# cnettel/cnF2freq

Measured on AMD Instinct MI355X. Metric: individual*marker fwd-bwd steps/sec (all 8 shift modes, forward+backward, dosage rows), higher is better.
Workload: dtype f64

## Files before the change

cnf2freq_amd/capi.py:

```python
import ctypes as C
import os

import numpy as np

_HERE = os.path.dirname(os.path.abspath(__file__))
LIB_PATH = os.environ.get("CNF2HIP_LIB") or os.path.join(_HERE, "libcnf2hip.so")

OUT_DEVICE, NO_DOSAGE, RAW_DOSAGE, NO_TIES, FULL_SPILL, MERGE_MODES, ACC_DEVICE, ACC_KEEP, XPOSE, LOG_PATHS = 1, 2, 4, 8, 16, 32, 64, 128, 256, 512
ACC_TABLE = 1024
ACC_LANES = 2048
TIES_GENERAL = 4096
UPDATE_PLAIN = 8192
UPDATE_BOTH_FLOWS = 1 << 16
UPDATE_ONE_SCOUT = 1 << 17
UPDATE_LITERAL_FINISH = 1 << 19
DETERMINISTIC = 16384
TURN_VALU = 32768
FLUSH_TINY = 1 << 20
ALL_STATES = 1 << 21
QTL_ADDITIVE = 1 << 22
QTL_ORIGIN_DEVICE = 1 << 23
QTL_REG_DEVICE = 1 << 28
QTL_IMPRINT = 1 << 25
QTL_STATE_DEVICE = 1 << 29
NO_UNIFORM_PACK = 1 << 26
NO_UNIFORM_PACK8 = 1 << 27
NO_LINE_RECORDS = 1 << 24
STATIC_JOBS = 1 << 18
MINFACTOR = float(np.float32(-1e15))
IGNORED = -1e30

SYMBOLS = [
    "cnf2_device_count", "cnf2_ctx_create", "cnf2_ctx_destroy", "cnf2_last_error", "cnf2_version",
    "cnf2_upload_map", "cnf2_upload_rows", "cnf2_update_rows", "cnf2_update_rows_device",
    "cnf2_upload_pedigree",
    "cnf2_window_info", "cnf2_sweep", "cnf2_sync", "cnf2_fwbw_store", "cnf2_locked_query",
    "cnf2_turn_scan", "cnf2_turn_scan_rows", "cnf2_state_posterior", "cnf2_haplos", "cnf2_infprobs", "cnf2_infprobs_rows", "cnf2_descendants", "cnf2_accumulate", "cnf2_sweep_accumulate", "cnf2_sweep_turn_scan", "cnf2_fixparents_scan", "cnf2_variances", "cnf2_variances_exact",
    "cnf2_snapshot_priors", "cnf2_update_pass", "cnf2_download_rows", "cnf2_download_accumulators", "cnf2_upload_accumulators", "cnf2_accumulator_ptrs", "cnf2_update_stats", "cnf2_update_stats_guided", "cnf2_addvariance", "cnf2_emission", "cnf2_emission_paths",
    "cnf2_selftest_lane_xor", "cnf2_last_kernel_ms", "cnf2_last_paths", "cnf2_workspace_bytes", "cnf2_reserve_accumulate", "cnf2_clock_probe", "cnf2_sweep_clock", "cnf2_stream",
    "cnf2_set_grid_reserve", "cnf2_set_batch_jobs", "cnf2_set_line_records", "cnf2_last_line_records", "cnf2_last_uniform_pack", "cnf2_last_uniform_pack8", "cnf2_window_table", "cnf2_update_pass_records", "cnf2_exchange_buffer", "cnf2_exchange_download", "cnf2_exchange_upload", "cnf2_exchange_read", "cnf2_exchange_write",
    "cnf2_packed_accumulator_doubles", "cnf2_packed_row_bytes", "cnf2_pack_accumulators", "cnf2_unpack_accumulators",
    "cnf2_pack_rows", "cnf2_unpack_rows",
    "cnf2_crossover_rows", "cnf2_sweep_crossovers", "cnf2_sweep_viterbi", "cnf2_sweep_sample",
    "cnf2_sweep_place", "cnf2_sweep_loo", "cnf2_loo_rows", "cnf2_sweep_origins", "cnf2_origin_rows",
    "cnf2_qtl_scan", "cnf2_sweep_qtl", "cnf2_set_qtl_columns", "cnf2_qtl_scan2", "cnf2_set_qtl2_columns", "cnf2_qtl_scanx", "cnf2_set_qtlx_columns",
    "cnf2_qtl_scan_em", "cnf2_set_qtlem_columns", "cnf2_qtl_scan_binary", "cnf2_set_qtlbin_columns",
    "cnf2_qtl_scan_surv", "cnf2_set_qtlsurv_columns", "cnf2_set_qtlsurv_blocks",
    "cnf2_qtl_scan_var", "cnf2_set_qtlvar_columns",
    "cnf2_qtl_scan_cof", "cnf2_set_qtlcof_columns", "cnf2_qtl_kept_rows",
    "cnf2_kinship_sums", "cnf2_qtl_scan_cols", "cnf2_qtl_scan_boot", "cnf2_qtl_scan_mv", "cnf2_set_qtlmv_groups",
    "cnf2_qtl_scan_imp", "cnf2_set_qtlimp_columns",
]


class Cnf2Error(RuntimeError):
    pass


_lib = None


def hip_runtimes():
    paths = set()
# ... 95 lines not shown
        L.cnf2_snapshot_priors.argtypes = [vp, vp]
        L.cnf2_update_pass.argtypes = [vp, i32, vp, vp, vp, vp, vp, C.c_double, C.c_double, vp, C.c_uint32]
        L.cnf2_download_rows.argtypes = [vp, i32, i32, vp, vp, vp]
        L.cnf2_download_accumulators.argtypes = [vp, vp, vp, vp]
        L.cnf2_upload_accumulators.argtypes = [vp, vp, vp, vp]
        L.cnf2_accumulator_ptrs.argtypes = [vp, vp, vp, vp]
        L.cnf2_update_stats.argtypes = [vp, vp]
        L.cnf2_update_stats_guided.argtypes = [vp, vp]
        L.cnf2_emission.argtypes = [vp, i32, i32, vp]
        L.cnf2_emission_paths.argtypes = [vp, i32, i32, vp]
        L.cnf2_selftest_lane_xor.argtypes = [vp, vp]
        L.cnf2_last_kernel_ms.argtypes = [vp, vp, i32]
        L.cnf2_last_paths.argtypes = [vp, vp, i32]
        L.cnf2_workspace_bytes.argtypes = [vp]
        L.cnf2_workspace_bytes.restype = C.c_size_t
        L.cnf2_clock_probe.argtypes = [vp, vp]
        L.cnf2_sweep_clock.argtypes = [vp, vp]
        L.cnf2_set_grid_reserve.argtypes = [vp, i32]
        L.cnf2_set_batch_jobs.argtypes = [vp, i32]
        L.cnf2_set_line_records.argtypes = [vp, i32]
        L.cnf2_last_line_records.argtypes = [vp, vp]
        L.cnf2_last_uniform_pack.argtypes = [vp, vp]
        L.cnf2_last_uniform_pack8.argtypes = [vp, vp]
        L.cnf2_window_table.argtypes = [vp, vp]
        L.cnf2_update_pass_records.argtypes = [vp, i32, vp, i32, vp, vp, C.c_double, C.c_double, vp, C.c_uint32]
        L.cnf2_exchange_buffer.argtypes = [vp, C.c_size_t, vp]
        L.cnf2_exchange_download.argtypes = [vp, vp, C.c_size_t]
        L.cnf2_exchange_upload.argtypes = [vp, vp, C.c_size_t]
        L.cnf2_exchange_read.argtypes = [vp, C.c_size_t, vp, C.c_size_t]
        L.cnf2_exchange_write.argtypes = [vp, C.c_size_t, vp, C.c_size_t]
        L.cnf2_packed_accumulator_doubles.argtypes = [vp]
        L.cnf2_packed_accumulator_doubles.restype = C.c_size_t
        L.cnf2_packed_row_bytes.argtypes = [vp]
        L.cnf2_packed_row_bytes.restype = C.c_size_t
        for f in (L.cnf2_pack_accumulators, L.cnf2_unpack_accumulators, L.cnf2_pack_rows, L.cnf2_unpack_rows):
            f.argtypes = [vp, vp, i32, vp]
        L.cnf2_stream.argtypes = [vp]
        L.cnf2_stream.restype = vp
        _lib = L
    return _lib


def _p(a):
    return a.ctypes.data_as(C.c_void_p)


# ... 131 lines not shown
        self._chk(self.L.cnf2_last_kernel_ms(self.h, _p(ms), 4), "cnf2_last_kernel_ms")
        return float(ms[0])

    def set_grid_reserve(self, blocks):
        self._chk(self.L.cnf2_set_grid_reserve(self.h, blocks), "cnf2_set_grid_reserve")

    def set_line_records(self, lines):
        self._chk(self.L.cnf2_set_line_records(self.h, lines), "cnf2_set_line_records")

    def last_line_records(self):
        out = np.zeros(4, np.int32)
        self._chk(self.L.cnf2_last_line_records(self.h, _p(out)), "cnf2_last_line_records")
        return dict(lines=int(out[0]), on_records=int(out[1]), fallback=int(out[2]), bytes=int(out[3]))

    def last_uniform_pack(self):
        out = np.zeros(2, np.int32)
        self._chk(self.L.cnf2_last_uniform_pack(self.h, _p(out)), "cnf2_last_uniform_pack")
        return dict(jobs=int(out[0]), groups=int(out[1]))

    def last_uniform_pack8(self):
        out = np.zeros(2, np.int32)
        self._chk(self.L.cnf2_last_uniform_pack8(self.h, _p(out)), "cnf2_last_uniform_pack8")
        return dict(eights=int(out[0]), jobs=int(out[1]))

    def set_batch_jobs(self, jobs):
        self._chk(self.L.cnf2_set_batch_jobs(self.h, jobs), "cnf2_set_batch_jobs")

    def workspace_bytes(self):
        return int(self.L.cnf2_workspace_bytes(self.h))

    def window_info(self, ind):
        out = np.zeros(17, np.int32)
        self._chk(self.L.cnf2_window_info(self.h, ind, _p(out)), "cnf2_window_info")
        return dict(shiftignore=int(out[0]), flag2ignore=int(out[1]), founder=int(out[2]),
                    slots=out[3:10].copy(), tie=out[10:17].copy())

    def fwbw_store(self, ind, chrom=0):
        mc = int(self.chromstarts[chrom + 1] - self.chromstarts[chrom])
        fw = np.zeros((8, mc, 3, 64))
        ff = np.zeros((8, mc, 3))
        self._chk(self.L.cnf2_fwbw_store(self.h, ind, chrom, _p(fw), _p(ff)), "cnf2_fwbw_store")
        return fw, ff

    def locked_query(self, ind, chrom, marker):
        v = np.zeros((8, 64, 128))
        self._chk(self.L.cnf2_locked_query(self.h, ind, chrom, marker, _p(v)), "cnf2_locked_query")
# ... 875 lines not shown
```

cnf2freq_amd/csrc/cnf2_capi.hip:

```cpp
#include "../../include/cnf2hip.h"

#include <hip/hip_runtime.h>
#include <math.h>
#include <cmath>
#include <stdarg.h>
#include <chrono>
#include <stdio.h>
#include <string.h>

#include <string>
#include <algorithm>
#include <vector>

#include "cnf2_device.h"
#include "cnf2_emission.h"
#include "cnf2_emtab.h"
#include "cnf2_plan.h"
#include "cnf2_qtl.h"
#include "cnf2_qtlplan.h"
#include "cnf2_qtl2.h"
#include "cnf2_qtlx.h"
#include "cnf2_qtlcof.h"
#include "cnf2_qtlem.h"
#include "cnf2_qtlbin.h"
// ... 76 lines not shown
    std::vector<Window> windows;
    DevBuf<Window>      d_windows;
    bool                windows_dirty = true;
    DevBuf<uint8_t>     d_rowflags;
    int                 fast_blocks_per_cu = 1;
    int                 uni_blocks_per_cu = 1;
    int                 reserve_blocks = 0;
    int                 batch_jobs = 0;

    int                  line_cap = -1;
    int32_t              last_lines[4] = {0, 0, 0, 0};
    int32_t              last_pack[2] = {0, 0};
    int32_t              last_pack8[2] = {0, 0};
    unsigned             windows_gen = 0;
    bool                 lines_valid = false;
    unsigned             lines_gen = 0;
    int                  lines_begin = 0, lines_n = 0, lines_cap = 0;
    int                  lines_fit = 1 << 30;
    std::vector<LineKey> h_lines;
    std::vector<int32_t> h_line_keys, h_line_hash;
    DevBuf<LineKey>      d_lines;
    DevBuf<int32_t>      d_line_keys;
    DevBuf<LineRec>      d_line_rec;

    DevBuf<Job>       d_jobs;
    DevBuf<PackedJob> d_pjobs;
    DevBuf<double>    d_spill;
    DevBuf<double>    d_factors, d_loglik, d_dosage;
    DevBuf<int32_t>   d_lexp;
    DevBuf<unsigned long long> d_clock;
    DevBuf<PackedJob> d_upjobs;
    DevBuf<int>       d_jobnext;
    DevBuf<double>    d_scratch;

    DevBuf<double>  d_xo_f;
    int             xo_blocks_per_cu = 1;
    DevBuf<double>  d_xo;
    DevBuf<double>  d_xo_sum;
    DevBuf<int32_t> d_xo_cnt;

    DevBuf<double>  d_vit_lm;
    DevBuf<uint8_t> d_vit_st;
    DevBuf<int32_t> d_vit_sh;

    DevBuf<uint8_t> d_smp_st;
    DevBuf<int32_t> d_smp_sh;
// ... 288 lines not shown

int cnf2_sync(cnf2_ctx* ctx)
{
    if (!ctx) return CNF2_ERR_ARG;
    HIP_TRY(ctx, hipStreamSynchronize(ctx->stream));
    return CNF2_OK;
}

int cnf2_upload_map(cnf2_ctx* ctx, const double* pos, int n_markers, const int32_t* chromstarts, int n_chrom,
                    const double* genrec)
{
    if (!ctx || !pos || !chromstarts || n_markers <= 0 || n_chrom <= 0) return fail(ctx, CNF2_ERR_ARG, "bad map arguments");
    if (chromstarts[0] != 0 || chromstarts[n_chrom] != n_markers)
        return fail(ctx, CNF2_ERR_ARG, "chromstarts must run from 0 to n_markers");
    for (int c = 0; c < n_chrom; c++)
        if (chromstarts[c + 1] <= chromstarts[c]) return fail(ctx, CNF2_ERR_ARG, "empty chromosome %d", c);
    HIP_TRY(ctx, hipSetDevice(ctx->device));
    if (ctx->n_markers != n_markers && (ctx->d_allele8 || ctx->d_sure || ctx->d_hw))
        return fail(ctx, CNF2_ERR_STATE, "marker count changed after rows were uploaded");
    ctx->qtl_rows_n = 0;
    ctx->n_markers = n_markers;
    ctx->n_chrom   = n_chrom;
    ctx->chromstarts.assign(chromstarts, chromstarts + n_chrom + 1);
    if (genrec) memcpy(ctx->genrec, genrec, sizeof(ctx->genrec));
    std::vector<double2> rho(n_markers);
    for (int m = 0; m < n_markers; m++) {
        double2 r = make_double2(0.0, 0.0);
        if (m + 1 < n_markers) {
            double dist = pos[m + 1] - pos[m];
            if (dist > 0) {
                r.x = 0.5 * (1.0 - exp(ctx->genrec[0] * dist));
                r.y = 0.5 * (1.0 - exp(ctx->genrec[1] * dist));
            }
        }
        rho[m] = r;
    }
    RC_TRY(ctx->d_rho.alloc(ctx, n_markers));
    HIP_TRY(ctx, hipMemcpy(ctx->d_rho, rho.data(), sizeof(double2) * n_markers, hipMemcpyHostToDevice));
    std::vector<double2> tq(n_markers);
    std::vector<double>  logk(n_chrom, 0.0);
    for (int c = 0; c < n_chrom; c++)
        for (int m = chromstarts[c]; m < chromstarts[c + 1]; m++) {
            tq[m] = make_double2(rho[m].x / (1.0 - rho[m].x), rho[m].y / (1.0 - rho[m].y));
            if (m + 1 < chromstarts[c + 1]) logk[c] += 4.0 * log1p(-rho[m].x) + 2.0 * log1p(-rho[m].y);
        }
    RC_TRY(ctx->d_tq.release(ctx));
// ... 335 lines not shown
        ctx->lines_n     = n;
        ctx->lines_cap   = cap;
        ctx->lines_valid = true;
    }
    *n_lines = (int)ctx->h_lines.size();
    return CNF2_OK;
}

static int sweep_impl(cnf2_ctx* ctx, int ind_begin, int ind_end, double* factors_out, double* loglik_out, double* dosage_out,
                      uint32_t flags, const SweepMode& mode)
{
    RC_TRY(ready(ctx));
    const int n_all = (int)ctx->windows.size();
    if (ind_begin < 0 || ind_end > n_all || ind_begin > ind_end) return fail(ctx, CNF2_ERR_ARG, "individual range out of bounds");
    const bool plain = mode.variant == SW_PLAIN;
    if (!plain) flags &= ~(uint32_t)(CNF2_MERGE_MODES | CNF2_XPOSE | CNF2_FLUSH_TINY | CNF2_NO_TIES | CNF2_RAW_DOSAGE);
    const bool want_dosage = !(flags & CNF2_NO_DOSAGE) && plain;
    if (!factors_out || !loglik_out || (want_dosage && !dosage_out)) return fail(ctx, CNF2_ERR_ARG, "output pointer is NULL");
    const int n = ind_end - ind_begin;
    if (n == 0) return CNF2_OK;
    HIP_TRY(ctx, hipSetDevice(ctx->device));

    if ((size_t)n * ctx->n_chrom > 0x7fffffff) return fail(ctx, CNF2_ERR_ARG, "too many jobs in one call");
    JobPlan      jp = job_plan(ctx, ind_begin, n, flags);
    const size_t n_fast = jp.n_fast, n_general = jp.jobs.size() - n_fast, n_packed = jp.pjobs.size();
    RC_TRY(ctx->d_jobs.ensure(ctx, jp.jobs.size() + 1));
    if (n_packed > 0) {
        RC_TRY(ctx->d_pjobs.ensure(ctx, n_packed));
        HIP_TRY(ctx, hipMemcpyAsync(ctx->d_pjobs, jp.pjobs.data(), sizeof(PackedJob) * n_packed, hipMemcpyHostToDevice, ctx->stream));
    }
    std::vector<PackedJob> ugroups;
    const std::vector<Job> jobs_planned = jp.jobs;
    auto group_and_upload = [&](const int32_t* keys) -> int {
        jp.jobs = jobs_planned;
        ugroups.clear();
        size_t n_single = n_fast;
        if (keys && !(flags & CNF2_NO_UNIFORM_PACK))
            ugroups = group_uniform_jobs(jp.jobs, n_fast, ctx->windows.data() + ind_begin, keys, &n_single);
        if (!jp.jobs.empty())
            HIP_TRY(ctx, hipMemcpyAsync(ctx->d_jobs, jp.jobs.data(), sizeof(Job) * jp.jobs.size(), hipMemcpyHostToDevice, ctx->stream));
        HIP_TRY(ctx, hipStreamSynchronize(ctx->stream));
        return CNF2_OK;
    };

    const int    mlen = longest_chrom(ctx);
    const size_t stride = spill_stride(mlen);
    int          grid_fast = 0, grid_gen = 0;
    size_t       free_b = 0, total_b = 0;
    HIP_TRY(ctx, hipMemGetInfo(&free_b, &total_b));
    size_t n_uniform = 0, n_on_records = 0;
    int    n_lines = 0;
    const bool uni_ok = !(flags & (CNF2_ALL_STATES | CNF2_FULL_SPILL | CNF2_XPOSE)) && (plain || mode.variant == SW_VITERBI);
    const int  want_lines = ctx->line_cap >= 0 ? std::min(ctx->line_cap, ctx->lines_fit) : ctx->lines_fit;
    auto count_uniform = [&]() {
        n_uniform = n_on_records = 0;
        const int32_t* keys = n_lines > 0 ? ctx->h_line_keys.data() : nullptr;
        for (size_t j = 0; j < n_fast; j++) {
            const int i = jp.jobs[j].ind;
            if (!slots_uniform(ctx->windows[ind_begin + i].flags)) continue;
            n_uniform++;
            if (keys && keys[2 * (size_t)i] >= 0) n_on_records++;
        }
    };
    memset(ctx->last_lines, 0, sizeof(ctx->last_lines));
    memset(ctx->last_pack, 0, sizeof(ctx->last_pack));
    memset(ctx->last_pack8, 0, sizeof(ctx->last_pack8));
    if (uni_ok) {
        if (n_fast > 0 && !(flags & CNF2_NO_LINE_RECORDS)) RC_TRY(prepare_lines(ctx, ind_begin, n, want_lines, &n_lines));
        count_uniform();
    }
    RC_TRY(group_and_upload(uni_ok && n_lines > 0 ? ctx->h_line_keys.data() : nullptr));
    const int fast_per_cu = n_uniform == 0       ? ctx->fast_blocks_per_cu
                            : n_uniform < n_fast ? std::max(ctx->fast_blocks_per_cu, ctx->uni_blocks_per_cu)
                                                 : ctx->uni_blocks_per_cu;
    if (!plan_sweep_grids(ctx->n_cu, fast_per_cu, ctx->blocks_per_cu, ctx->reserve_blocks, std::max(n_fast, n_packed),
                          n_general, free_b, ctx->d_spill.cap * sizeof(double), mlen, &grid_fast, &grid_gen))
        return fail(ctx, CNF2_ERR_NOMEM, "a chromosome of %d markers needs %zu MB of spill per block, %zu MB free", mlen,
                    spill_block_bytes(mlen) >> 20, free_b >> 20);
    RC_TRY(ctx->d_spill.ensure(ctx, (size_t)(grid_fast + grid_gen) * CNF2_WAVES_PER_BLOCK * stride));

    double *d_f, *d_l, *d_d = nullptr;
    const size_t nf = (size_t)n * ctx->n_chrom * 8, nl = (size_t)n * ctx->n_chrom, nd = (size_t)n * ctx->n_markers * 3;
    if (flags & CNF2_OUT_DEVICE) {
        d_f = factors_out;
        d_l = loglik_out;
        d_d = dosage_out;
    } else {
        RC_TRY(ctx->d_factors.ensure(ctx, nf));
        RC_TRY(ctx->d_loglik.ensure(ctx, nl));
        if (want_dosage) RC_TRY(ctx->d_dosage.ensure(ctx, nd));
        d_f = ctx->d_factors;
        d_l = ctx->d_loglik;
        d_d = ctx->d_dosage;
    }

    if (n_on_records == 0) n_lines = 0;
    if (n_lines > 0) {
        const size_t line_bytes = (size_t)ctx->n_markers * LINE_VALUES * 2 * sizeof(LineRec);
        if ((size_t)n_lines * line_bytes > ctx->d_line_rec.cap * sizeof(LineRec)) {
            HIP_TRY(ctx, hipMemGetInfo(&free_b, &total_b));
            const size_t fit = (ctx->d_line_rec.cap * sizeof(LineRec) + free_b / 2) / line_bytes;
            if (fit < (size_t)n_lines) {
                ctx->lines_fit = (int)fit;
                RC_TRY(prepare_lines(ctx, ind_begin, n, std::min(want_lines, ctx->lines_fit), &n_lines));
                count_uniform();
                if (n_on_records == 0) n_lines = 0;
                RC_TRY(group_and_upload(n_lines > 0 ? ctx->h_line_keys.data() : nullptr));
            }
        }
        if (n_lines > 0) RC_TRY(ctx->d_line_rec.ensure(ctx, (size_t)n_lines * ctx->n_markers * LINE_VALUES * 2));
    }
    ctx->last_lines[0] = n_lines;
    ctx->last_lines[1] = n_lines > 0 ? (int32_t)n_on_records : 0;
    ctx->last_lines[2] = (int32_t)n_uniform - ctx->last_lines[1];
    ctx->last_lines[3] = (int32_t)std::min<size_t>((size_t)n_lines * ctx->n_markers * LINE_VALUES * 2 * sizeof(LineRec), 0x7fffffff);
    const size_t n_groups = n_lines > 0 ? ugroups.size() : 0;
    ctx->last_pack[0] = (int32_t)(4 * n_groups);
    ctx->last_pack[1] = (int32_t)n_groups;
    const int pack_cap = std::min(grid_fast, resident_blocks(ctx->n_cu, ctx->uni_blocks_per_cu, ctx->reserve_blocks));
    size_t    n_eights = 0;
    if (n_groups > 0) {
        if (!(flags & CNF2_NO_UNIFORM_PACK8))
            n_eights = pair_uniform_groups(ugroups, ctx->windows.data() + ind_begin, (size_t)pack_cap * CNF2_WAVES_PER_BLOCK);
        RC_TRY(ctx->d_upjobs.ensure(ctx, ugroups.size()));
        HIP_TRY(ctx, hipMemcpyAsync(ctx->d_upjobs, ugroups.data(), sizeof(PackedJob) * ugroups.size(), hipMemcpyHostToDevice, ctx->stream));
        HIP_TRY(ctx, hipStreamSynchronize(ctx->stream));
    }
    ctx->last_pack8[0] = (int32_t)n_eights;
    ctx->last_pack8[1] = (int32_t)(8 * n_eights);

    KernelParams p;
    base_params(ctx, &p);
    p.windows      = ctx->d_windows + ind_begin;
    p.jobs         = ctx->d_jobs;
    p.n_jobs       = (int)n_fast;
    p.spill        = ctx->d_spill;
    p.spill_stride = stride;
    p.factors      = d_f;
    p.loglik       = d_l;
    p.dosage       = d_d;
    p.flags        = (want_dosage ? 0 : KP_NO_DOSAGE) | ((flags & CNF2_RAW_DOSAGE) ? KP_RAW_DOSAGE : 0) |
              ((flags & CNF2_NO_TIES) ? KP_NO_TIES : 0);
    if (flags & CNF2_STATIC_JOBS) p.job_next = nullptr;
    int follow_per_cu = 0;
    switch (mode.variant) {
    case SW_CROSSOVERS:
        p.flags  = 0;
        p.xo     = mode.xo;
        p.xo_sum = mode.xo_sum;
        p.xo_cnt = mode.xo_cnt;
// ... 24 lines not shown
        follow_per_cu = ctx->fast_blocks_per_cu;
        break;
    case SW_ORIGINS:
        p.flags  = KP_NO_DOSAGE;
        p.org    = mode.org;
        p.obits  = mode.obits;
        p.xo_cnt = mode.xo_cnt;
        follow_per_cu = ctx->fast_blocks_per_cu;
        break;
    default: break;
    }
    if (flags & CNF2_LOG_PATHS) {
        RC_TRY(ctx->d_pathlog.ensure(ctx, nl));
        HIP_TRY(ctx, hipMemsetAsync(ctx->d_pathlog, 0xff, nl * sizeof(int32_t), ctx->stream));
        p.path_log     = ctx->d_pathlog;
        ctx->pathlog_n = (int)nl;
    }
    const bool half = !(flags & CNF2_FULL_SPILL);
    auto likelihoods_to_scratch = [&](KernelParams* q) {
        q->factors = ctx->d_xo_f;
        q->loglik  = ctx->d_xo_f + (size_t)n * ctx->n_chrom * 8;
    };

    HIP_TRY(ctx, hipEventRecord(ctx->ev0, ctx->stream));
    if (n_general > 0) {
        KernelParams pt = p;
        HIP_TRY(ctx, hipStreamWaitEvent(ctx->stream2, ctx->ev0, 0));
        pt.jobs   = ctx->d_jobs + n_fast;
        pt.n_jobs = (int)n_general;
        if (pt.job_next) pt.job_next = ctx->d_jobnext + 1;
        pt.spill  = ctx->d_spill + (size_t)((n_fast > 0 || n_packed > 0) ? grid_fast : 0) * CNF2_WAVES_PER_BLOCK * stride;
        if (flags & CNF2_FLUSH_TINY) pt.flags |= KP_FLUSH_TINY;
        if (!plain) pt.flags = KP_NO_DOSAGE;
        if (flags & (CNF2_FULL_SPILL | CNF2_TIES_GENERAL | CNF2_FLUSH_TINY))
            HIP_TRY(ctx, launch_fb(pt, grid_gen, SW_PLAIN, ctx->stream2));
        else HIP_TRY(ctx, launch_fb_fast(pt, grid_gen, {SW_PLAIN, true, false, true}, ctx->stream2));
        if (!plain) {
            KernelParams px = pt;
            likelihoods_to_scratch(&px);
            const int gx = std::min(resident_blocks(ctx->n_cu, follow_per_cu, ctx->reserve_blocks), grid_gen);
            if (mode.variant == SW_CROSSOVERS) HIP_TRY(ctx, launch_fb(px, gx, SW_CROSSOVERS, ctx->stream2));
            else HIP_TRY(ctx, launch_fb_fast(px, gx, {mode.variant, half}, ctx->stream2));
        }
        HIP_TRY(ctx, hipEventRecord(ctx->ev2, ctx->stream2));
    }
    if (n_packed > 0) {
// ... 66 lines not shown
}

int cnf2_last_line_records(cnf2_ctx* ctx, int32_t* out)
{
    if (!ctx || !out) return fail(ctx, CNF2_ERR_ARG, "bad arguments");
    memcpy(out, ctx->last_lines, sizeof(ctx->last_lines));
    return CNF2_OK;
}

int cnf2_last_uniform_pack(cnf2_ctx* ctx, int32_t* out)
{
    if (!ctx || !out) return fail(ctx, CNF2_ERR_ARG, "bad arguments");
    memcpy(out, ctx->last_pack, sizeof(ctx->last_pack));
    return CNF2_OK;
}

int cnf2_last_uniform_pack8(cnf2_ctx* ctx, int32_t* out)
{
    if (!ctx || !out) return fail(ctx, CNF2_ERR_ARG, "bad arguments");
    memcpy(out, ctx->last_pack8, sizeof(ctx->last_pack8));
    return CNF2_OK;
}

int cnf2_last_paths(cnf2_ctx* ctx, int32_t* paths_out, int n)
{
    if (!ctx || !paths_out || n < 0) return fail(ctx, CNF2_ERR_ARG, "bad path arguments");
    if (!ctx->d_pathlog || n > ctx->pathlog_n) return fail(ctx, CNF2_ERR_STATE, "no sweep with CNF2_LOG_PATHS covers %d jobs", n);
    HIP_TRY(ctx, hipSetDevice(ctx->device));
    HIP_TRY(ctx, hipStreamSynchronize(ctx->stream));
    HIP_TRY(ctx, hipMemcpy(paths_out, ctx->d_pathlog, (size_t)n * sizeof(int32_t), hipMemcpyDeviceToHost));
    return CNF2_OK;
}

int cnf2_last_kernel_ms(cnf2_ctx* ctx, float* kernel_ms, int n)
{
    if (!ctx || !kernel_ms || n < 1) return CNF2_ERR_ARG;
    if (!ctx->timed) return fail(ctx, CNF2_ERR_STATE, "no sweep has been launched");
    HIP_TRY(ctx, hipEventSynchronize(ctx->ev1));
    float ms = 0;
    HIP_TRY(ctx, hipEventElapsedTime(&ms, ctx->ev0, ctx->ev1));
    kernel_ms[0] = ms;
    for (int i = 1; i < n; i++) kernel_ms[i] = 0;
    return CNF2_OK;
}

int cnf2_sweep_clock(cnf2_ctx* ctx, double* mhz_out)
// ... 1626 lines not shown
    return CNF2_OK;
}

static size_t todo_chunk(size_t n_rec, size_t chrom_len, size_t markers_upto)
{
    const size_t n1 = n_rec * chrom_len * 4, n3 = n_rec * markers_upto;
    size_t       want = n1 > n3 ? n1 : n3;
    if (want < 4096) want = 4096;
    const size_t cap = (size_t)1 << 26;
    return want < cap ? want : cap;
}

#ifdef CNF2_X_GUIDED_ROUNDS
#define TODO_LISTS 3
#else
#define TODO_LISTS 2
#endif
static size_t todo_doubles(size_t chunk) { return chunk * 3 * TODO_LISTS + chunk / 256 + 8; }

static int batched_setup(cnf2_ctx* ctx, int ind_begin, int n, uint32_t flags, size_t row_doubles, size_t part_need, Batched* b)
{
    b->list = job_plan(ctx, ind_begin, n, flags & CNF2_NO_TIES);
    const std::vector<Job>& jobs = b->list.jobs;
    RC_TRY(ctx->d_jobs.ensure(ctx, jobs.size() + 1));
    HIP_TRY(ctx, hipMemcpy(ctx->d_jobs, jobs.data(), sizeof(Job) * jobs.size(), hipMemcpyHostToDevice));
    b->max_len = longest_chrom(ctx);
    size_t free_b = 0, total_b = 0;
    HIP_TRY(ctx, hipMemGetInfo(&free_b, &total_b));
    const size_t held_b = (ctx->d_spill.cap + ctx->d_wbuf.cap) * sizeof(double);
    b->plan = plan_batches(ctx->n_cu, ctx->fast_blocks_per_cu, ctx->reserve_blocks, free_b, held_b, b->max_len, row_doubles, jobs.size(), ctx->batch_jobs, part_need, ctx->d_part.cap);
    if (b->plan.fit == BATCH_NO_SPILL) return fail(ctx, CNF2_ERR_NOMEM, "not enough memory for the spill of one block");
    return ctx->d_spill.ensure(ctx, (size_t)b->plan.grid_cap * CNF2_WAVES_PER_BLOCK * spill_stride(b->max_len));
}

enum : uint32_t { ACC_RESERVE_ONLY = 1u << 31 };
enum : uint32_t { PLACE_SWEEP_LIKELIHOODS = 1u << 30, PLACE_OWN_LIKELIHOODS = 1u << 29 };

int cnf2_sweep_accumulate(cnf2_ctx* ctx, int ind_begin, int ind_end, const int32_t* descendants, double* factors_out,
                          double* loglik_out, double* dosage_out, double* infprobs, double* haplobase,
                          double* haplocount, double* homozyg, uint32_t flags)
{
    RC_TRY(ready(ctx));
    const int n_all = (int)ctx->windows.size();
    const bool out_dev = (flags & CNF2_OUT_DEVICE) != 0, acc_dev = (flags & CNF2_ACC_DEVICE) != 0;
    const bool acc_given = infprobs && haplobase && haplocount && homozyg;
    const bool acc_none = !infprobs && !haplobase && !haplocount && !homozyg;
// ... 933 lines not shown
```

cnf2freq_amd/csrc/cnf2_emtab.h:

```cpp
#ifndef CNF2_EMTAB_H
#define CNF2_EMTAB_H

#include "cnf2_emission.h"

#if defined(__HIP_DEVICE_COMPILE__)
#define CNF2_SCHED_FENCE() __builtin_amdgcn_sched_barrier(0)
#else
#define CNF2_SCHED_FENCE() ((void)0)
#endif

namespace cnf2 {

struct PartCfg {
    uint32_t par, tr, ot;
    int      P, f, firstpar;
    bool     root_attop;
    int      force_par = -1, force_tr = -1, force_ot = -1;
};

CNF2_HD void match_affine(int inmv, int mf, double sf, double* Bv, double* K, double* C, int* mv)
{
    bool miss;
    if (inmv == 0) {
        *mv  = mf;
// ... 363 lines not shown
    const double pm1 = (fl_par & SLOT_RESTRICT0) ? 0.0 : 1.0;
    uint32_t bits = 0;
    if (!bzero && wq0 + wq1 != 0.0) bits |= LR_LIVE;
#pragma unroll
    for (int kind = 1; kind < 3; kind++)
#pragma unroll
        for (int sp = 0; sp < 2; sp++) {
            const double w = (sp ? wq1 : wq0) + pm1 * (sp ? wq0 : wq1);
#pragma unroll
            for (int bo = 0; bo < 2; bo++)
#pragma unroll
                for (int bt = 0; bt < 2; bt++) {
                    double g0, g1, q0, q1;
                    leaf_value(Lt, bt, kind, &g0, &g1);
                    leaf_value(Lo, bo, 1, &q0, &q1);
                    const bool on = !bzero && w != 0.0 && (g0 != 0.0 || g1 != 0.0) && (q0 != 0.0 || q1 != 0.0);
                    if (on) bits |= 1u << ((kind - 1) * 8 + sp * 4 + bo * 2 + bt);
                }
        }
    r->bits   = bits;
    r->pad[0] = r->pad[1] = r->pad[2] = 0;
}

CNF2_HD constexpr bool packed_reads_unrestricted(int e) { return (e & 3) == 0; }
template <bool CLASSES, bool PACKED = false, class Out>
CNF2_HD void emtab_part_rec(int P, int f, const Slot& root, const LineRec& r, Out&& out, double cw[2])
{
    const SlotDirect rv(root);
    const int    mf = rv.allele(f);
    const double sf = rv.sure(f), so_r = rv.sure(f ^ 1);
    const double base_r = 1.0 - sf;
    const double msv_r  = (mf != 0) ? sf : 0.0;
    cw[0] = rv.w(f ^ 0);
    cw[1] = rv.w(f ^ 1);
    if (base_r == 0.0) cw[0] = cw[1] = 0.0;
    const double u0 = P ? 1.0 - so_r : base_r;
    const double u1 = P ? so_r : msv_r;
    const double alpha = u0 * r.Bp;
    const double beta  = CNF2_FMA2(u0, r.Cp, u1, r.Kp);
#ifdef CNF2_LINEREC_PER_ENTRY
    const double ga = CNF2_FMA2(alpha, r.t0, beta, r.t1), gb = CNF2_FMA2(beta, r.t1, alpha, r.t0);
#pragma unroll
    for (int e = 0; e < 8; e++) out(0, e, ((r.bits & LR_LIVE) ? 1.0 : 0.0) * (r.oo * ga));
    if (CLASSES) {
#pragma unroll
        for (int e = 0; e < 8; e++) {
            out(1, e, (double)((r.bits >> e) & 1) * (r.oo * ((e & 1) ? ga : gb)));
            out(2, e, (double)((r.bits >> (8 + e)) & 1) * (r.oo * ga));
        }
    }
    return;
#endif
    const double va = r.oo * CNF2_FMA2(alpha, r.t0, beta, r.t1);
    const double v0 = (r.bits & LR_LIVE) ? va : 0.0;
#pragma unroll
    for (int e = 0; e < 8; e++)
        if (!PACKED || packed_reads_unrestricted(e)) out(0, e, v0);
    if (CLASSES) {
        const double vb = r.oo * CNF2_FMA2(beta, r.t1, alpha, r.t0);
#pragma unroll
        for (int e = 0; e < 8; e++) {
            out(1, e, ((r.bits >> e) & 1) ? ((e & 1) ? va : vb) : 0.0);
            out(2, e, ((r.bits >> (8 + e)) & 1) ? va : 0.0);
        }
    }
}

CNF2_HD void make_part(const Window& w, int part, PartCfg* c, int32_t* row_par, int32_t* row_tr, int32_t* row_ot)
{
    const int  P = part >> 2, f = (part >> 1) & 1, firstpar = part & 1;
    const bool hi = P != 0, fp = firstpar != 0;
    c->P = P;
    c->f = f;
    c->firstpar   = firstpar;
    const uint32_t fa = hi ? w.flags[5] : w.flags[2], fb = hi ? w.flags[6] : w.flags[3];
    const int32_t  ra = hi ? w.row[5] : w.row[2], rb = hi ? w.row[6] : w.row[3];
    const int32_t  rp = hi ? w.row[4] : w.row[1];
    c->par        = hi ? w.flags[4] : w.flags[1];
    c->tr         = fp ? fb : fa;
    c->ot         = fp ? fa : fb;
    c->root_attop = (w.flags[0] & SLOT_FOUNDER) != 0;
    const int32_t rt = fp ? rb : ra, ro = fp ? ra : rb;
    *row_par = rp < 0 ? 0 : rp;
    *row_tr  = rt < 0 ? 0 : rt;
    *row_ot  = ro < 0 ? 0 : ro;
}
// ... 23 lines not shown
```

cnf2freq_amd/csrc/cnf2_plan.h:

```cpp
#ifndef CNF2_PLAN_H
#define CNF2_PLAN_H

#include <stddef.h>
#include <stdint.h>

#include <algorithm>
#include <vector>

#include "../../include/cnf2hip.h"
#include "cnf2_emission.h"
#include "cnf2_job.h"
#include "cnf2_window.h"

namespace cnf2 {

inline std::vector<int> chrom_order(const int32_t* chromstarts, int n_chrom)
{
    std::vector<int> o(n_chrom);
    for (int c = 0; c < n_chrom; c++) o[c] = c;
    std::stable_sort(o.begin(), o.end(), [&](int a, int b) {
        return chromstarts[a + 1] - chromstarts[a] > chromstarts[b + 1] - chromstarts[b];
    });
    return o;
}
// ... 131 lines not shown
                seconds.push_back(g);
                open = e;
            }
        }
        b = e;
    }
    size_t n8 = firsts.size();
    if (waves > 0 && n8 >= waves) n8 = n8 / waves * waves;
    if (n8 == 0) return 0;
    std::vector<uint8_t>   paired(groups.size(), 0);
    std::vector<PackedJob> out;
    out.reserve(groups.size());
    for (size_t k = 0; k < n8; k++) {
        out.push_back(groups[firsts[k]]);
        out.push_back(groups[seconds[k]]);
        paired[firsts[k]] = paired[seconds[k]] = 1;
    }
    for (size_t g = 0; g < groups.size(); g++)
        if (!paired[g]) out.push_back(groups[g]);
    groups.swap(out);
    return n8;
}

constexpr size_t PLAN_SPILL_ROW = 528;
inline size_t spill_stride(int max_len) { return (size_t)max_len * PLAN_SPILL_ROW; }
inline size_t spill_block_bytes(int max_len) { return (size_t)CNF2_WAVES_PER_BLOCK * spill_stride(max_len) * sizeof(double); }

inline int resident_blocks(int n_cu, int per_cu, int reserve_blocks) { return std::max(1, n_cu * per_cu - reserve_blocks); }
inline int grid_for(size_t n_jobs, int cap)
{
    const size_t blocks = (n_jobs + CNF2_WAVES_PER_BLOCK - 1) / CNF2_WAVES_PER_BLOCK;
    return (int)std::min(blocks, (size_t)cap);
}

constexpr double PLAN_SWEEP_SPILL_SHARE = 0.6;

inline bool plan_sweep_grids(int n_cu, int fast_per_cu, int gen_per_cu, int reserve_blocks, size_t n_fast, size_t n_general,
                             size_t free_bytes, size_t held_bytes, int max_len, int* grid_fast, int* grid_gen)
{
    const size_t budget = (size_t)((double)(free_bytes + held_bytes) * PLAN_SWEEP_SPILL_SHARE);
    const size_t per_blk = spill_block_bytes(max_len);
    const size_t max_blks = budget / per_blk;
    if (max_blks < 1) return false;
    int gf = (int)std::min((size_t)grid_for(n_fast, resident_blocks(n_cu, fast_per_cu, reserve_blocks)), max_blks);
    int gg = (int)std::min((size_t)grid_for(n_general, resident_blocks(n_cu, gen_per_cu, reserve_blocks)), max_blks);
    if (n_fast > 0 && n_general > 0)
// ... 63 lines not shown
```

include/cnf2hip.h:

```cpp
#ifndef CNF2HIP_H
#define CNF2HIP_H

#include <stddef.h>
#include <stdint.h>

#ifdef __cplusplus
extern "C" {
#endif

#define CNF2_NUMTYPES   64
#define CNF2_NUMSHIFTS  8
#define CNF2_NUMPATHS   128
#define CNF2_MINFACTOR  (-1e15f)
#define CNF2_IGNORED    (-1e30)

enum {
    CNF2_OK            = 0,
    CNF2_ERR_NO_DEVICE = -1,
    CNF2_ERR_ARG       = -2,
    CNF2_ERR_STATE     = -3,
    CNF2_ERR_HIP       = -4,
    CNF2_ERR_NOMEM     = -5
};

// ... 216 lines not shown
int cnf2_update_stats_guided(cnf2_ctx *ctx, uint64_t *out8);
int cnf2_download_accumulators(cnf2_ctx *ctx, double *infprobs, double *haplobase, double *haplocount);
int cnf2_accumulator_ptrs(cnf2_ctx *ctx, double **infprobs, double **haplobase, double **haplocount);
int cnf2_upload_accumulators(cnf2_ctx *ctx, const double *infprobs, const double *haplobase, const double *haplocount);

int cnf2_emission(cnf2_ctx *ctx, int ind, int marker, double *e_out);
int cnf2_emission_paths(cnf2_ctx *ctx, int ind, int marker, double *e_out);

int cnf2_selftest_lane_xor(cnf2_ctx *ctx, double *out384);

int    cnf2_last_kernel_ms(cnf2_ctx *ctx, float *kernel_ms, int n);
int    cnf2_last_paths(cnf2_ctx *ctx, int32_t *paths_out, int n);
size_t cnf2_workspace_bytes(cnf2_ctx *ctx);
int    cnf2_clock_probe(cnf2_ctx *ctx, double *mhz_out);
int    cnf2_sweep_clock(cnf2_ctx *ctx, double *mhz_out);
void  *cnf2_stream(cnf2_ctx *ctx);
int    cnf2_set_grid_reserve(cnf2_ctx *ctx, int blocks);
int    cnf2_set_batch_jobs(cnf2_ctx *ctx, int jobs);
int    cnf2_set_line_records(cnf2_ctx *ctx, int lines);
int    cnf2_last_line_records(cnf2_ctx *ctx, int32_t *out);
int    cnf2_last_uniform_pack(cnf2_ctx *ctx, int32_t *out);
int    cnf2_last_uniform_pack8(cnf2_ctx *ctx, int32_t *out);

#ifdef __cplusplus
}
#endif
#endif
```

Baseline: 5.389 billion.

## Cache host job plan across sweep calls and use bitmask select in emtab

```diff
diff --git a/cnf2freq_amd/capi.py b/cnf2freq_amd/capi.py
--- a/cnf2freq_amd/capi.py
+++ b/cnf2freq_amd/capi.py
@@ -38,7 +38,7 @@
     "cnf2_turn_scan", "cnf2_turn_scan_rows", "cnf2_state_posterior", "cnf2_haplos", "cnf2_infprobs", "cnf2_infprobs_rows", "cnf2_descendants", "cnf2_accumulate", "cnf2_sweep_accumulate", "cnf2_sweep_turn_scan", "cnf2_fixparents_scan", "cnf2_variances", "cnf2_variances_exact",
     "cnf2_snapshot_priors", "cnf2_update_pass", "cnf2_download_rows", "cnf2_download_accumulators", "cnf2_upload_accumulators", "cnf2_accumulator_ptrs", "cnf2_update_stats", "cnf2_update_stats_guided", "cnf2_addvariance", "cnf2_emission", "cnf2_emission_paths",
     "cnf2_selftest_lane_xor", "cnf2_last_kernel_ms", "cnf2_last_paths", "cnf2_workspace_bytes", "cnf2_reserve_accumulate", "cnf2_clock_probe", "cnf2_sweep_clock", "cnf2_stream",
-    "cnf2_set_grid_reserve", "cnf2_set_batch_jobs", "cnf2_set_line_records", "cnf2_last_line_records", "cnf2_last_uniform_pack", "cnf2_last_uniform_pack8", "cnf2_window_table", "cnf2_update_pass_records", "cnf2_exchange_buffer", "cnf2_exchange_download", "cnf2_exchange_upload", "cnf2_exchange_read", "cnf2_exchange_write",
+    "cnf2_set_grid_reserve", "cnf2_set_batch_jobs", "cnf2_set_line_records", "cnf2_last_line_records", "cnf2_last_uniform_pack", "cnf2_last_uniform_pack8", "cnf2_last_plan_reused", "cnf2_last_plan_ms", "cnf2_window_table", "cnf2_update_pass_records", "cnf2_exchange_buffer", "cnf2_exchange_download", "cnf2_exchange_upload", "cnf2_exchange_read", "cnf2_exchange_write",
     "cnf2_packed_accumulator_doubles", "cnf2_packed_row_bytes", "cnf2_pack_accumulators", "cnf2_unpack_accumulators",
     "cnf2_pack_rows", "cnf2_unpack_rows",
     "cnf2_crossover_rows", "cnf2_sweep_crossovers", "cnf2_sweep_viterbi", "cnf2_sweep_sample",
@@ -180,6 +180,9 @@
         L.cnf2_last_line_records.argtypes = [vp, vp]
         L.cnf2_last_uniform_pack.argtypes = [vp, vp]
         L.cnf2_last_uniform_pack8.argtypes = [vp, vp]
+        L.cnf2_last_plan_reused.argtypes = [vp]
+        L.cnf2_last_plan_ms.argtypes = [vp]
+        L.cnf2_last_plan_ms.restype = C.c_float
         L.cnf2_window_table.argtypes = [vp, vp]
         L.cnf2_update_pass_records.argtypes = [vp, i32, vp, i32, vp, vp, C.c_double, C.c_double, vp, C.c_uint32]
         L.cnf2_exchange_buffer.argtypes = [vp, C.c_size_t, vp]
@@ -357,6 +360,12 @@
         out = np.zeros(2, np.int32)
         self._chk(self.L.cnf2_last_uniform_pack8(self.h, _p(out)), "cnf2_last_uniform_pack8")
         return dict(eights=int(out[0]), jobs=int(out[1]))
+
+    def last_plan_reused(self):
+        return bool(self.L.cnf2_last_plan_reused(self.h))
+
+    def last_plan_ms(self):
+        return float(self.L.cnf2_last_plan_ms(self.h))
 
     def set_batch_jobs(self, jobs):
         self._chk(self.L.cnf2_set_batch_jobs(self.h, jobs), "cnf2_set_batch_jobs")
diff --git a/cnf2freq_amd/csrc/cnf2_capi.hip b/cnf2freq_amd/csrc/cnf2_capi.hip
--- a/cnf2freq_amd/csrc/cnf2_capi.hip
+++ b/cnf2freq_amd/csrc/cnf2_capi.hip
@@ -122,6 +122,15 @@
     DevBuf<LineKey>      d_lines;
     DevBuf<int32_t>      d_line_keys;
     DevBuf<LineRec>      d_line_rec;
+
+    unsigned               map_gen = 0;
+    bool                   plan_valid = false;
+    PlanKey                plan_key;
+    JobPlan                plan_list;
+    std::vector<PackedJob> plan_fours, plan_groups;
+    size_t                 plan_n_uniform = 0, plan_n_on_records = 0, plan_n_eights = 0;
+    int                    last_plan_reused = 0;
+    float                  last_plan_ms = 0.f;
 
     DevBuf<Job>       d_jobs;
     DevBuf<PackedJob> d_pjobs;
@@ -456,6 +465,7 @@
     ctx->n_markers = n_markers;
     ctx->n_chrom   = n_chrom;
     ctx->chromstarts.assign(chromstarts, chromstarts + n_chrom + 1);
+    ctx->map_gen++;
     if (genrec) memcpy(ctx->genrec, genrec, sizeof(ctx->genrec));
     std::vector<double2> rho(n_markers);
     for (int m = 0; m < n_markers; m++) {
@@ -837,57 +847,75 @@
     HIP_TRY(ctx, hipSetDevice(ctx->device));
 
     if ((size_t)n * ctx->n_chrom > 0x7fffffff) return fail(ctx, CNF2_ERR_ARG, "too many jobs in one call");
-    JobPlan      jp = job_plan(ctx, ind_begin, n, flags);
-    const size_t n_fast = jp.n_fast, n_general = jp.jobs.size() - n_fast, n_packed = jp.pjobs.size();
-    RC_TRY(ctx->d_jobs.ensure(ctx, jp.jobs.size() + 1));
-    if (n_packed > 0) {
-        RC_TRY(ctx->d_pjobs.ensure(ctx, n_packed));
-        HIP_TRY(ctx, hipMemcpyAsync(ctx->d_pjobs, jp.pjobs.data(), sizeof(PackedJob) * n_packed, hipMemcpyHostToDevice, ctx->stream));
-    }
-    std::vector<PackedJob> ugroups;
-    const std::vector<Job> jobs_planned = jp.jobs;
-    auto group_and_upload = [&](const int32_t* keys) -> int {
-        jp.jobs = jobs_planned;
-        ugroups.clear();
-        size_t n_single = n_fast;
+    const auto t_plan = std::chrono::steady_clock::now();
+    ctx->last_plan_reused = 0;
+    memset(ctx->last_lines, 0, sizeof(ctx->last_lines));
+    memset(ctx->last_pack, 0, sizeof(ctx->last_pack));
+    memset(ctx->last_pack8, 0, sizeof(ctx->last_pack8));
+
+    int        n_lines = 0;
+    const bool uni_ok = !(flags & (CNF2_ALL_STATES | CNF2_FULL_SPILL | CNF2_XPOSE)) && (plain || mode.variant == SW_VITERBI);
+    int        want_lines = ctx->line_cap >= 0 ? std::min(ctx->line_cap, ctx->lines_fit) : ctx->lines_fit;
+    if (uni_ok && !(flags & CNF2_NO_LINE_RECORDS)) RC_TRY(prepare_lines(ctx, ind_begin, n, want_lines, &n_lines));
+
+    PlanKey key;
+    key.windows_gen       = ctx->windows_gen;
+    key.map_gen           = ctx->map_gen;
+    key.ind_begin         = ind_begin;
+    key.n                 = n;
+    key.flags             = flags & PLAN_KEY_FLAGS;
+    key.uniform_mode      = uni_ok ? 1 : 0;
+    key.reserve_blocks    = ctx->reserve_blocks;
+    key.uni_blocks_per_cu = ctx->uni_blocks_per_cu;
+    auto key_lines = [&]() {
+        key.n_lines   = n_lines;
+        key.lines_cap = want_lines;
+        key.lines_fit = ctx->lines_fit;
+    };
+    key_lines();
+    JobPlan&                jp = ctx->plan_list;
+    std::vector<PackedJob>& fours = ctx->plan_fours;
+    auto build_jobs = [&]() -> int {
+        ctx->plan_valid = false;
+        jp = job_plan(ctx, ind_begin, n, flags);
+        RC_TRY(ctx->d_jobs.ensure(ctx, jp.jobs.size() + 1));
+        if (!jp.pjobs.empty()) {
+            RC_TRY(ctx->d_pjobs.ensure(ctx, jp.pjobs.size()));
+            HIP_TRY(ctx, hipMemcpyAsync(ctx->d_pjobs, jp.pjobs.data(), sizeof(PackedJob) * jp.pjobs.size(), hipMemcpyHostToDevice, ctx->stream));
+        }
+        const int32_t* keys = uni_ok && n_lines > 0 ? ctx->h_line_keys.data() : nullptr;
+        ctx->plan_n_uniform = ctx->plan_n_on_records = 0;
+        for (size_t j = 0; uni_ok && j < jp.n_fast; j++) {
+            const int i = jp.jobs[j].ind;
+            if (!slots_uniform(ctx->windows[ind_begin + i].flags)) continue;
+            ctx->plan_n_uniform++;
+            if (keys && keys[2 * (size_t)i] >= 0) ctx->plan_n_on_records++;
+        }
+        fours.clear();
+        size_t n_single = jp.n_fast;
         if (keys && !(flags & CNF2_NO_UNIFORM_PACK))
-            ugroups = group_uniform_jobs(jp.jobs, n_fast, ctx->windows.data() + ind_begin, keys, &n_single);
+            fours = group_uniform_jobs(jp.jobs, jp.n_fast, ctx->windows.data() + ind_begin, keys, &n_single);
         if (!jp.jobs.empty())
             HIP_TRY(ctx, hipMemcpyAsync(ctx->d_jobs, jp.jobs.data(), sizeof(Job) * jp.jobs.size(), hipMemcpyHostToDevice, ctx->stream));
         HIP_TRY(ctx, hipStreamSynchronize(ctx->stream));
         return CNF2_OK;
     };
+#ifdef CNF2_NO_PLAN_CACHE
+    ctx->plan_valid = false;
+#endif
+    bool same_jobs = ctx->plan_valid && plan_key_same_jobs(ctx->plan_key, key);
+    if (!same_jobs) RC_TRY(build_jobs());
+    const size_t n_fast = jp.n_fast, n_general = jp.jobs.size() - n_fast, n_packed = jp.pjobs.size();
 
     const int    mlen = longest_chrom(ctx);
     const size_t stride = spill_stride(mlen);
     int          grid_fast = 0, grid_gen = 0;
     size_t       free_b = 0, total_b = 0;
     HIP_TRY(ctx, hipMemGetInfo(&free_b, &total_b));
-    size_t n_uniform = 0, n_on_records = 0;
-    int    n_lines = 0;
-    const bool uni_ok = !(flags & (CNF2_ALL_STATES | CNF2_FULL_SPILL | CNF2_XPOSE)) && (plain || mode.variant == SW_VITERBI);
-    const int  want_lines = ctx->line_cap >= 0 ? std::min(ctx->line_cap, ctx->lines_fit) : ctx->lines_fit;
-    auto count_uniform = [&]() {
-        n_uniform = n_on_records = 0;
-        const int32_t* keys = n_lines > 0 ? ctx->h_line_keys.data() : nullptr;
-        for (size_t j = 0; j < n_fast; j++) {
-            const int i = jp.jobs[j].ind;
-            if (!slots_uniform(ctx->windows[ind_begin + i].flags)) continue;
-            n_uniform++;
-            if (keys && keys[2 * (size_t)i] >= 0) n_on_records++;
-        }
-    };
-    memset(ctx->last_lines, 0, sizeof(ctx->last_lines));
-    memset(ctx->last_pack, 0, sizeof(ctx->last_pack));
-    memset(ctx->last_pack8, 0, sizeof(ctx->last_pack8));
-    if (uni_ok) {
-        if (n_fast > 0 && !(flags & CNF2_NO_LINE_RECORDS)) RC_TRY(prepare_lines(ctx, ind_begin, n, want_lines, &n_lines));
-        count_uniform();
-    }
-    RC_TRY(group_and_upload(uni_ok && n_lines > 0 ? ctx->h_line_keys.data() : nullptr));
-    const int fast_per_cu = n_uniform == 0       ? ctx->fast_blocks_per_cu
-                            : n_uniform < n_fast ? std::max(ctx->fast_blocks_per_cu, ctx->uni_blocks_per_cu)
-                                                 : ctx->uni_blocks_per_cu;
+    const size_t n_uniform0 = ctx->plan_n_uniform;
+    const int fast_per_cu = n_uniform0 == 0       ? ctx->fast_blocks_per_cu
+                            : n_uniform0 < n_fast ? std::max(ctx->fast_blocks_per_cu, ctx->uni_blocks_per_cu)
+                                                  : ctx->uni_blocks_per_cu;
     if (!plan_sweep_grids(ctx->n_cu, fast_per_cu, ctx->blocks_per_cu, ctx->reserve_blocks, std::max(n_fast, n_packed),
                           n_general, free_b, ctx->d_spill.cap * sizeof(double), mlen, &grid_fast, &grid_gen))
         return fail(ctx, CNF2_ERR_NOMEM, "a chromosome of %d markers needs %zu MB of spill per block, %zu MB free", mlen,
@@ -909,7 +937,7 @@
         d_d = ctx->d_dosage;
     }
 
-    if (n_on_records == 0) n_lines = 0;
+    if (ctx->plan_n_on_records == 0) n_lines = 0;
     if (n_lines > 0) {
         const size_t line_bytes = (size_t)ctx->n_markers * LINE_VALUES * 2 * sizeof(LineRec);
         if ((size_t)n_lines * line_bytes > ctx->d_line_rec.cap * sizeof(LineRec)) {
@@ -917,30 +945,43 @@
             const size_t fit = (ctx->d_line_rec.cap * sizeof(LineRec) + free_b / 2) / line_bytes;
             if (fit < (size_t)n_lines) {
                 ctx->lines_fit = (int)fit;
-                RC_TRY(prepare_lines(ctx, ind_begin, n, std::min(want_lines, ctx->lines_fit), &n_lines));
-                count_uniform();
-                if (n_on_records == 0) n_lines = 0;
-                RC_TRY(group_and_upload(n_lines > 0 ? ctx->h_line_keys.data() : nullptr));
+                want_lines     = std::min(want_lines, ctx->lines_fit);
+                RC_TRY(prepare_lines(ctx, ind_begin, n, want_lines, &n_lines));
+                key_lines();
+                same_jobs = false;
+                RC_TRY(build_jobs());
+                if (ctx->plan_n_on_records == 0) n_lines = 0;
             }
         }
         if (n_lines > 0) RC_TRY(ctx->d_line_rec.ensure(ctx, (size_t)n_lines * ctx->n_markers * LINE_VALUES * 2));
     }
+    const size_t n_uniform = ctx->plan_n_uniform, n_on_records = ctx->plan_n_on_records;
     ctx->last_lines[0] = n_lines;
     ctx->last_lines[1] = n_lines > 0 ? (int32_t)n_on_records : 0;
     ctx->last_lines[2] = (int32_t)n_uniform - ctx->last_lines[1];
     ctx->last_lines[3] = (int32_t)std::min<size_t>((size_t)n_lines * ctx->n_markers * LINE_VALUES * 2 * sizeof(LineRec), 0x7fffffff);
-    const size_t n_groups = n_lines > 0 ? ugroups.size() : 0;
+    const size_t n_groups = n_lines > 0 ? fours.size() : 0;
     ctx->last_pack[0] = (int32_t)(4 * n_groups);
     ctx->last_pack[1] = (int32_t)n_groups;
     const int pack_cap = std::min(grid_fast, resident_blocks(ctx->n_cu, ctx->uni_blocks_per_cu, ctx->reserve_blocks));
-    size_t    n_eights = 0;
-    if (n_groups > 0) {
-        if (!(flags & CNF2_NO_UNIFORM_PACK8))
-            n_eights = pair_uniform_groups(ugroups, ctx->windows.data() + ind_begin, (size_t)pack_cap * CNF2_WAVES_PER_BLOCK);
-        RC_TRY(ctx->d_upjobs.ensure(ctx, ugroups.size()));
-        HIP_TRY(ctx, hipMemcpyAsync(ctx->d_upjobs, ugroups.data(), sizeof(PackedJob) * ugroups.size(), hipMemcpyHostToDevice, ctx->stream));
-        HIP_TRY(ctx, hipStreamSynchronize(ctx->stream));
-    }
+    key.pack_cap = pack_cap;
+    if (!(same_jobs && plan_key_same(ctx->plan_key, key))) {
+        std::vector<PackedJob>& ugroups = ctx->plan_groups;
+        ctx->plan_valid    = false;
+        ctx->plan_n_eights = 0;
+        ugroups.clear();
+        if (n_groups > 0) {
+            ugroups = fours;
+            if (!(flags & CNF2_NO_UNIFORM_PACK8))
+                ctx->plan_n_eights = pair_uniform_groups(ugroups, ctx->windows.data() + ind_begin, (size_t)pack_cap * CNF2_WAVES_PER_BLOCK);
+            RC_TRY(ctx->d_upjobs.ensure(ctx, ugroups.size()));
+            HIP_TRY(ctx, hipMemcpyAsync(ctx->d_upjobs, ugroups.data(), sizeof(PackedJob) * ugroups.size(), hipMemcpyHostToDevice, ctx->stream));
+            HIP_TRY(ctx, hipStreamSynchronize(ctx->stream));
+        }
+        ctx->plan_key   = key;
+        ctx->plan_valid = true;
+    } else ctx->last_plan_reused = 1;
+    const size_t n_eights = ctx->plan_n_eights;
     ctx->last_pack8[0] = (int32_t)n_eights;
     ctx->last_pack8[1] = (int32_t)(8 * n_eights);
 
@@ -1011,6 +1052,7 @@
         q->loglik  = ctx->d_xo_f + (size_t)n * ctx->n_chrom * 8;
     };
 
+    ctx->last_plan_ms = std::chrono::duration<float, std::milli>(std::chrono::steady_clock::now() - t_plan).count();
     HIP_TRY(ctx, hipEventRecord(ctx->ev0, ctx->stream));
     if (n_general > 0) {
         KernelParams pt = p;
@@ -1123,6 +1165,10 @@
     return CNF2_OK;
 }
 
+int cnf2_last_plan_reused(cnf2_ctx* ctx) { return ctx ? ctx->last_plan_reused : 0; }
+
+float cnf2_last_plan_ms(cnf2_ctx* ctx) { return ctx ? ctx->last_plan_ms : 0.f; }
+
 int cnf2_last_paths(cnf2_ctx* ctx, int32_t* paths_out, int n)
 {
     if (!ctx || !paths_out || n < 0) return fail(ctx, CNF2_ERR_ARG, "bad path arguments");
@@ -2795,6 +2841,7 @@
 {
     b->list = job_plan(ctx, ind_begin, n, flags & CNF2_NO_TIES);
     const std::vector<Job>& jobs = b->list.jobs;
+    ctx->plan_valid = false;
     RC_TRY(ctx->d_jobs.ensure(ctx, jobs.size() + 1));
     HIP_TRY(ctx, hipMemcpy(ctx->d_jobs, jobs.data(), sizeof(Job) * jobs.size(), hipMemcpyHostToDevice));
     b->max_len = longest_chrom(ctx);
diff --git a/cnf2freq_amd/csrc/cnf2_emtab.h b/cnf2freq_amd/csrc/cnf2_emtab.h
--- a/cnf2freq_amd/csrc/cnf2_emtab.h
+++ b/cnf2freq_amd/csrc/cnf2_emtab.h
@@ -1,5 +1,7 @@
 #ifndef CNF2_EMTAB_H
 #define CNF2_EMTAB_H
+
+#include <string.h>
 
 #include "cnf2_emission.h"
 
@@ -409,6 +411,23 @@
     r->pad[0] = r->pad[1] = r->pad[2] = 0;
 }
 
+CNF2_HD double keep_if_bit(uint32_t bits, int e, double v)
+{
+#if defined(CNF2_EMTAB_SELECT)
+    return ((bits >> e) & 1) ? v : 0.0;
+#elif defined(__HIP_DEVICE_COMPILE__)
+    const int m = __builtin_amdgcn_sbfe((int)bits, (unsigned)e, 1u);
+    return __hiloint2double(__double2hiint(v) & m, __double2loint(v) & m);
+#else
+    uint64_t u;
+    memcpy(&u, &v, sizeof(u));
+    u &= (uint64_t)0 - (uint64_t)((bits >> e) & 1);
+    double r;
+    memcpy(&r, &u, sizeof(r));
+    return r;
+#endif
+}
+
 CNF2_HD constexpr bool packed_reads_unrestricted(int e) { return (e & 3) == 0; }
 template <bool CLASSES, bool PACKED = false, class Out>
 CNF2_HD void emtab_part_rec(int P, int f, const Slot& root, const LineRec& r, Out&& out, double cw[2])
@@ -439,7 +458,7 @@
     return;
 #endif
     const double va = r.oo * CNF2_FMA2(alpha, r.t0, beta, r.t1);
-    const double v0 = (r.bits & LR_LIVE) ? va : 0.0;
+    const double v0 = keep_if_bit(r.bits, 16, va);
 #pragma unroll
     for (int e = 0; e < 8; e++)
         if (!PACKED || packed_reads_unrestricted(e)) out(0, e, v0);
@@ -447,8 +466,8 @@
         const double vb = r.oo * CNF2_FMA2(beta, r.t1, alpha, r.t0);
 #pragma unroll
         for (int e = 0; e < 8; e++) {
-            out(1, e, ((r.bits >> e) & 1) ? ((e & 1) ? va : vb) : 0.0);
-            out(2, e, ((r.bits >> (8 + e)) & 1) ? va : 0.0);
+            out(1, e, keep_if_bit(r.bits, e, (e & 1) ? va : vb));
+            out(2, e, keep_if_bit(r.bits, 8 + e, va));
         }
     }
 }
diff --git a/cnf2freq_amd/csrc/cnf2_plan.h b/cnf2freq_amd/csrc/cnf2_plan.h
--- a/cnf2freq_amd/csrc/cnf2_plan.h
+++ b/cnf2freq_amd/csrc/cnf2_plan.h
@@ -177,6 +177,30 @@
     return n8;
 }
 
+struct PlanKey {
+    unsigned windows_gen = 0, map_gen = 0;
+    int      ind_begin = 0, n = 0;
+    uint32_t flags = 0;
+    int      uniform_mode = 0;
+    int      n_lines = 0, lines_cap = 0, lines_fit = 0;
+    int      pack_cap = 0, reserve_blocks = 0, uni_blocks_per_cu = 0;
+};
+constexpr uint32_t PLAN_KEY_FLAGS = CNF2_MERGE_MODES | CNF2_FULL_SPILL | CNF2_FLUSH_TINY | CNF2_NO_TIES | CNF2_NO_UNIFORM_PACK |
+                                    CNF2_NO_UNIFORM_PACK8 | CNF2_NO_LINE_RECORDS | CNF2_ALL_STATES | CNF2_XPOSE;
+
+inline bool plan_key_same_jobs(const PlanKey& a, const PlanKey& b)
+{
+    const uint32_t pairing = CNF2_NO_UNIFORM_PACK8;
+    return a.windows_gen == b.windows_gen && a.map_gen == b.map_gen && a.ind_begin == b.ind_begin && a.n == b.n &&
+           (a.flags & PLAN_KEY_FLAGS & ~pairing) == (b.flags & PLAN_KEY_FLAGS & ~pairing) && a.uniform_mode == b.uniform_mode &&
+           a.n_lines == b.n_lines && a.lines_cap == b.lines_cap && a.lines_fit == b.lines_fit;
+}
+inline bool plan_key_same(const PlanKey& a, const PlanKey& b)
+{
+    return plan_key_same_jobs(a, b) && (a.flags & PLAN_KEY_FLAGS) == (b.flags & PLAN_KEY_FLAGS) && a.pack_cap == b.pack_cap &&
+           a.reserve_blocks == b.reserve_blocks && a.uni_blocks_per_cu == b.uni_blocks_per_cu;
+}
+
 constexpr size_t PLAN_SPILL_ROW = 528;
 inline size_t spill_stride(int max_len) { return (size_t)max_len * PLAN_SPILL_ROW; }
 inline size_t spill_block_bytes(int max_len) { return (size_t)CNF2_WAVES_PER_BLOCK * spill_stride(max_len) * sizeof(double); }
diff --git a/include/cnf2hip.h b/include/cnf2hip.h
--- a/include/cnf2hip.h
+++ b/include/cnf2hip.h
@@ -262,6 +262,9 @@
 int    cnf2_last_uniform_pack(cnf2_ctx *ctx, int32_t *out);
 int    cnf2_last_uniform_pack8(cnf2_ctx *ctx, int32_t *out);
 
+int    cnf2_last_plan_reused(cnf2_ctx *ctx);
+float  cnf2_last_plan_ms(cnf2_ctx *ctx);
+
 #ifdef __cplusplus
 }
 #endif
```

Result: faster. 5.773 billion (median of 6 runs) (+7.1%).
